# OndrejSladky/kmercamel

Hardware: NVIDIA B200
Metric: distinct k-mers/sec for `compute` (k=31, canonical, device-timed) (higher is better)
Workload: dtype u64

## Files before the change

kmercamel_b200/csrc/engine.cuh:

```cuda
#pragma once
#include "exec.cuh"
#include "kword.cuh"
#include "sort.cuh"
#ifdef KC_HOST_EMUL
#include <algorithm>
#endif

template <int L> struct NodeView {
    const KWord<L> *first;
    const KWord<L> *last;
    u32 n, N;
    int k;
    bool complements;
    KC_HD u32 mirror(u32 v) const { return v < n ? v + n : v - n; }
    KC_HD KWord<L> first_kmer(u32 v) const { return v < n ? first[v] : kmer_reverse_complement(last[v - n], k); }
    KC_HD KWord<L> last_kmer(u32 v) const { return v < n ? last[v] : kmer_reverse_complement(first[v - n], k); }
};

struct PathState {
    u32 *edge_from;
    u32 *edge_to;
    u8 *ovl;
    u32 *chain_head;
    u32 *chain_tail;
};

static const int KC_META_SHIFT = 27;
static const u64 KC_ROLE_P = 1ULL << 36;

template <int L> KC_HD KWord<L + 1> tuple_make(const KWord<L> &key, u64 meta) {
    KWord<L + 1> t;
    t.w[0] = meta << KC_META_SHIFT;
#pragma unroll
    for (int i = 0; i < L; ++i) t.w[i + 1] = key.w[i];
    return t;
}
template <int LT> KC_HD KWord<LT - 1> tuple_key(const KWord<LT> &t) {
    KWord<LT - 1> k;
#pragma unroll
    for (int i = 0; i < LT - 1; ++i) k.w[i] = t.w[i + 1];
    return k;
}
template <int LT> KC_HD bool tuple_is_prefix(const KWord<LT> &t) { return (t.w[0] >> (36 + KC_META_SHIFT)) & 1; }
template <int LT> KC_HD u32 tuple_part(const KWord<LT> &t) { return (u32) (t.w[0] >> (32 + KC_META_SHIFT)) & 15u; }
template <int LT> KC_HD u32 tuple_node(const KWord<LT> &t) {
    u32 id = (u32) (t.w[0] >> KC_META_SHIFT);
    return tuple_is_prefix(t) ? ~id : id;
}

template <int LT> KC_HD u64 tuple_lower_bound(const KWord<LT> *T, u64 lo, u64 hi, const KWord<LT> &probe) {
    while (lo < hi) {
        u64 mid = (lo + hi) >> 1;
        if (T[mid] < probe) lo = mid + 1;
        else hi = mid;
    }
    return lo;
}

#ifdef __CUDACC__
template <int LL> void exec_sort(CudaExec &ex, KWord<LL> *a, KWord<LL> *b, u64 n, int key_bits) { kc_sort<LL>(ex, a, b, n, key_bits); }
#endif
#ifdef KC_HOST_EMUL
template <int LL> void exec_sort(HostExec &, KWord<LL> *a, KWord<LL> *, u64 n, int) {
    std::sort(a, a + n, [](const KWord<LL> &x, const KWord<LL> &y) { return x < y; });
}
#endif

template <int L> struct LevelCtx {
    NodeView<L> nv;
    PathState st;
    const KWord<L + 1> *T;
    u64 nt;
    int d;
    u32 batch;
    u32 *head_w;
    u32 *tail_w;
    u64 *stamp;
    u8 *prim;
    const u8 *ban_flag;
    const u32 *ban_i, *ban_j;
    u32 n_bans;
    bool check_cycles;
};

template <int L> struct SimulatePairFn {
    LevelCtx<L> c;
    const u32 *group_pstart;

    KC_HD bool banned(u32 i, u32 j) const {
        if (!c.ban_flag[i]) return false;
        for (u32 b = 0; b < c.n_bans; ++b)
            if (c.ban_i[b] == i && c.ban_j[b] == j) return true;
        return false;
    }
    KC_HD bool owns_suffix(u32 v, const KWord<L> &ka, const KWord<L> &kb) const {
        if (c.d == 0) return true;
        KWord<L> s = kmer_suffix(c.nv.last_kmer(v), c.d);
        return s == ka || s == kb;
    }
    KC_HD bool owns_prefix(u32 v, const KWord<L> &ka, const KWord<L> &kb) const {
        if (c.d == 0) return true;
        KWord<L> p = kmer_prefix(c.nv.first_kmer(v), c.nv.k, c.d);
        return p == ka || p == kb;
    }
    KC_HD void link(u32 x, u32 y, u64 stampv, u8 primary, const KWord<L> &ka, const KWord<L> &kb) const {
        c.st.edge_from[x] = y;
        c.st.edge_to[y] = x;
        c.st.ovl[x] = (u8) c.d;
        c.stamp[x] = stampv;
        c.prim[x] = primary;
        u32 h = c.head_w[x], t = c.tail_w[y];
        if (owns_suffix(t, ka, kb)) c.head_w[t] = h;
        if (owns_prefix(h, ka, kb)) c.tail_w[h] = t;
    }

    KC_HD void operator()(u64 g) const {
        const KWord<L + 1> *T = c.T;
        const u64 p_beg = group_pstart[g];
        const KWord<L> ka = tuple_key(T[p_beg]);
        KWord<L> kb = ka;
        bool two = false;
        if (c.nv.complements) {
            kb = kmer_reverse_complement(ka, c.d);
            if (kb < ka) return;
            two = kb != ka;
        }
        const u64 meta_max = (1ULL << 37) - 1;
        const u64 s_beg = tuple_lower_bound(T, (u64) 0, p_beg, tuple_make(ka, 0));
        const u64 s_end = p_beg;
        const u64 pa_end = tuple_lower_bound(T, p_beg, c.nt, tuple_make(ka, meta_max));
        u64 s2_beg = 0, s2_end = 0, p2_beg = 0, p2_end = 0;
        if (two) {
            s2_beg = tuple_lower_bound(T, (u64) 0, c.nt, tuple_make(kb, 0));
            s2_end = tuple_lower_bound(T, s2_beg, c.nt, tuple_make(kb, KC_ROLE_P));
            p2_beg = s2_end;
            p2_end = tuple_lower_bound(T, p2_beg, c.nt, tuple_make(kb, meta_max));
        }
        u64 ca = p_beg, cb = p2_beg;
        for (u32 part = 0; part < 16; ++part) {
            u64 ra0 = ca;
            while (ca < pa_end && tuple_part(T[ca]) == part) ++ca;
            u64 ra1 = ca;
            u64 rb0 = cb;
            while (cb < p2_end && tuple_part(T[cb]) == part) ++cb;
            u64 rb1 = cb;
            if (ra0 == ra1 && rb0 == rb1) continue;
            u64 fa = ra0, fb = rb0;
            u64 ia = s_beg, ib = s2_beg;
            while (true) {
                u32 va = (ia < s_end && fa < ra1) ? tuple_node(T[ia]) : KC_NONE;
                u32 vb = (ib < s2_end && fb < rb1) ? tuple_node(T[ib]) : KC_NONE;
                if (va == KC_NONE && vb == KC_NONE) break;
                u32 i;
                u64 *front;
                u64 rend;
                if (va < vb) {
                    i = va;
                    ++ia;
                    front = &fa;
                    rend = ra1;
                } else {
                    i = vb;
                    ++ib;
                    front = &fb;
                    rend = rb1;
                }
                if (c.st.edge_from[i] != KC_NONE) continue;
                while (*front < rend && c.st.edge_to[tuple_node(T[*front])] != KC_NONE) ++*front;
                for (u64 q = *front; q < rend; ++q) {
                    u32 j = tuple_node(T[q]);
                    if (c.st.edge_to[j] != KC_NONE) continue;
                    if (c.check_cycles) {
                        if (c.nv.complements && j == c.nv.mirror(i)) continue;
                        if (j == c.head_w[i]) continue;
                        if (banned(i, j)) continue;
                    }
                    u64 stampv = ((u64) part << 32) | i;
                    link(i, j, stampv, 1, ka, kb);
                    if (c.nv.complements) link(c.nv.mirror(j), c.nv.mirror(i), stampv, 0, ka, kb);
                    break;
                }
            }
        }
    }
};

#ifdef __CUDACC__
#include <cooperative_groups.h>
__global__ void __launch_bounds__(256) kc_doubling_kernel(u32 *jump_a, u32 *jump_b, u32 *fin_a, u32 *fin_b, u64 *max_a, u64 *max_b, u32 ne, int rounds,
                                                          u32 *active , const u32 *ne_dev ) {
    cooperative_groups::grid_group grid = cooperative_groups::this_grid();
    if (ne_dev) ne = *ne_dev;
    u32 *ja = jump_a, *jb = jump_b, *fa = fin_a, *fb = fin_b;
    u64 *ma = max_a, *mb = max_b;
    const u32 stride = gridDim.x * blockDim.x;
    int it = 0;
    for (; it < rounds; ++it) {
        bool any = false;
        for (u32 r = blockIdx.x * blockDim.x + threadIdx.x; r < ne; r += stride) {
            const u32 j = ja[r];
            if (j == KC_NONE) {
                jb[r] = KC_NONE;
                fb[r] = fa[r];
                mb[r] = ma[r];
            } else {
                any = true;
                jb[r] = ja[j];
                fb[r] = fa[j];
                const u64 m1 = ma[r], m2 = ma[j];
                mb[r] = m1 > m2 ? m1 : m2;
            }
        }
        if (__syncthreads_or(any) && threadIdx.x == 0) atomicOr(&active[it % 3], 1u);
        if (blockIdx.x == 0 && threadIdx.x == 0) active[(it + 1) % 3] = 0;
        grid.sync();
        u32 *t = ja; ja = jb; jb = t;
        t = fa; fa = fb; fb = t;
        u64 *m = ma; ma = mb; mb = m;
        const u32 more = *reinterpret_cast<volatile u32 *>(&active[it % 3]);
        if (!more) {
            ++it;
            break;
        }
    }
    if (ja != jump_a) {
        grid.sync();
        for (u32 r = blockIdx.x * blockDim.x + threadIdx.x; r < ne; r += stride) {
            jump_a[r] = ja[r];
            fin_a[r] = fa[r];
            max_a[r] = ma[r];
        }
    }
}
#endif

#include "small_engine.cuh"

struct EngineStats {
    u64 levels_run = 0, tuples_sorted = 0, groups = 0, edges = 0, ban_rounds = 0, bans = 0;
};

template <class Exec, int L> struct Engine {
    Exec &ex;
    NodeView<L> nv;
    PathState st;
    bool strict;
    bool lower_bound;
    bool use_small = true;
    bool fast_levels = true;
    int small_threads_opt = 0;
    EngineStats stats;

    u32 *live_s = nullptr, *live_p = nullptr;
    u32 *list_buf[4] = {nullptr, nullptr, nullptr, nullptr};
    int list_gen = 0;
    u64 n_s = 0, n_p = 0;
    u32 *head_w, *tail_w, *slot_of;
    u64 *stamp;
    u8 *prim, *ban_flag;
    u32 *ban_i, *ban_j, *ban_ctr;
    static const u32 BAN_CAP = 1u << 20;

    Engine(Exec &e, const NodeView<L> &v, bool strict_, bool lower_bound_) : ex(e), nv(v), strict(strict_), lower_bound(lower_bound_) {}

    const u32 *n_dev = nullptr;
    u32 *small_status = nullptr, *small_masks = nullptr;

    void alloc_state() {
        const u64 N = nv.N;
        st.edge_from = ex.template alloc<u32>(N);
        st.edge_to = ex.template alloc<u32>(N);
        st.ovl = ex.template alloc<u8>(N);
        st.chain_head = ex.template alloc<u32>(N);
        st.chain_tail = ex.template alloc<u32>(N);
        head_w = ex.template alloc<u32>(N);
        tail_w = ex.template alloc<u32>(N);
        slot_of = ex.template alloc<u32>(N);
        stamp = ex.template alloc<u64>(N);
        prim = ex.template alloc<u8>(N);
        ban_flag = ex.template alloc<u8>(N);
        ban_i = ex.template alloc<u32>(BAN_CAP);
        ban_j = ex.template alloc<u32>(BAN_CAP);
        ban_ctr = ex.template alloc<u32>(4);
    }

    void init_state() {
        alloc_state();
        const u64 N = nv.N;
        PathState s = st;
        u8 *bf = ban_flag;
        u32 *bc = ban_ctr;
        ex.for_each(N, [=] KC_HD_LAMBDA(u64 v) {
            s.edge_from[v] = KC_NONE;
            s.edge_to[v] = KC_NONE;
            s.ovl[v] = 255;
            bf[v] = 0;
            s.chain_head[v] = (u32) v;
            s.chain_tail[v] = (u32) v;
            if (v < 4) bc[v] = 0;
        });
        if (N < 4) ex.fill_bytes(ban_ctr, 0, 16);
        n_s = n_p = N;
    }

    void run() {
        for (int d = nv.k - 1; d >= 0; --d) {
            const u64 done = lower_bound ? 0 : (nv.complements ? 2 : 1);
            if (n_s <= done) break;
            if (run_small(d)) break;
            run_level(d);
        }
    }

    u32 *small_out = nullptr;
    int small_d = 0;

    void check_small() {
#ifdef __CUDACC__
        if constexpr (Exec::is_device) {
            if (!small_out) return;
            u32 h[KC_SMALL_STATUS_WORDS];
            ex.read_n(small_out, h, KC_SMALL_STATUS_WORDS);
            small_out = nullptr;
            apply_small_status(h);
        }
#endif
    }

    void apply_small_status(const u32 *h) {
        if (std::getenv("KC_TRACE")) {
            std::fprintf(stderr, "[kc_trace] small engine: n_s=%llu n_p=%llu levels=%u groups=%u edges=%u ban_rounds=%u bans=%u; clocks per level (* = run):",
                         (unsigned long long) n_s, (unsigned long long) n_p, h[1], h[2], h[3], h[4], h[5]);
            for (int dd = small_d; dd >= 0; --dd) std::fprintf(stderr, " d%d=%u%s", dd, h[8 + dd] & 0x7FFFFFFFu, (h[8 + dd] >> 31) ? "*" : "");
            std::fprintf(stderr, "; phases: stage+mask=%u tuples=%u sort=%u groups=%u replay=%u validate+commit=%u lists=%u writeback=%u\n", h[136], h[137],
                         h[138], h[139], h[140], h[141], h[142], h[143]);
        }
        if (h[0]) KC_THROW(KC_ERR_INTERNAL, "ban list overflow");
        stats.levels_run += h[1];
        stats.groups += h[2];
        stats.edges += h[3];
        stats.ban_rounds += h[4];
        stats.bans += h[5];
    }

    bool run_small(int d) {
#ifdef __CUDACC__
        if constexpr (Exec::is_device) {
            if (!use_small || lower_bound || n_s + n_p > SmallCfg<L>::T) return false;
            if (!live_s) {
                u32 *a = ex.template alloc<u32>(n_s), *b = ex.template alloc<u32>(n_p);
                ex.for_each(nv.N, [=] KC_HD_LAMBDA(u64 i) {
                    a[i] = (u32) i;
                    b[i] = (u32) i;
                });
                live_s = a;
                live_p = b;
            }
            SmallEngineArgs<L> a;
            a.nv = nv;
            a.st = st;
            a.live_s_a = live_s;
            a.live_p_a = live_p;
            a.live_s_b = ex.template alloc<u32>(n_s);
            a.live_p_b = ex.template alloc<u32>(n_p);
            a.n_s = (u32) n_s;
            a.n_p = (u32) n_p;
            a.head_w = head_w;
            a.tail_w = tail_w;
            a.slot_of = slot_of;
            a.stamp = stamp;
            a.prim = prim;
            a.ban_flag = ban_flag;
            a.ban_i = ban_i;
            a.ban_j = ban_j;
            a.ban_cap = BAN_CAP;
            a.d_start = d;
            a.strict = strict;
            u32 *lvl_mask;
            if (n_dev) {
                a.out = small_status;
                lvl_mask = small_masks;
            } else {
                a.out = ex.template alloc<u32>(KC_SMALL_STATUS_WORDS + kc_small_mask_words(n_s, n_p) + 4 * (n_s + n_p));
                lvl_mask = a.out + KC_SMALL_STATUS_WORDS;
                ex.fill_bytes(a.out, 0, (KC_SMALL_STATUS_WORDS + kc_small_mask_words(n_s, n_p)) * 4);
            }
            a.n_dev = n_dev;
            a.lvl_mask_in = lvl_mask;
            a.end_mask_s_a = lvl_mask + 4;
            a.end_mask_p_a = a.end_mask_s_a + 4 * n_s;
            a.end_mask_s_b = a.end_mask_p_a + 4 * n_p;
            a.end_mask_p_b = a.end_mask_s_b + 4 * n_s;
            const int mask_smem = (int) (SmallCfg<L>::T * sizeof(KWord<L + 1>));
            static KcDevOnce once;
            once.run([&](int) {
                KC_CUDA(cudaFuncSetAttribute(kc_small_engine_kernel<L>, cudaFuncAttributeMaxDynamicSharedMemorySize,
                                             (int) SmallCfg<L>::SMEM));
                KC_CUDA(cudaFuncSetAttribute(kc_small_level_mask_kernel<L>, cudaFuncAttributeMaxDynamicSharedMemorySize, mask_smem));
            });
            {
                typename Exec::Scope sc(ex, KP_SMALL_ENGINE, 0);
                const u32 per_cta = kc_small_mask_levels_per_cta<L>((u32) n_s, (u32) n_p);
                kc_small_level_mask_kernel<L><<<(unsigned) kc_div_up((u64) d + 1, per_cta), 256, mask_smem, ex.stream>>>(nv, live_s, live_p, (u32) n_s, (u32) n_p, d,
                                                                                                                      lvl_mask, a.end_mask_s_a, a.end_mask_p_a, n_dev);
                ++ex.launches;
            }
            {
                typename Exec::Scope sc(ex, KP_SMALL_ENGINE, 0);
                const u64 nt0 = n_s + n_p;
                const unsigned small_threads = small_threads_opt ? (unsigned) small_threads_opt
                                               : n_dev || (nt0 > 128 && nt0 <= 256) || nt0 > 512 ? 512u : 256u;
                kc_small_engine_kernel<L><<<1, small_threads, SmallCfg<L>::SMEM, ex.stream>>>(a);
            }
            ++ex.launches;
            KC_CUDA(cudaGetLastError());
            small_out = n_dev ? nullptr : a.out;
            small_d = d;
            return true;
        }
#endif
        (void) d;
        return false;
    }

    void run_level(int d) {
        typedef KWord<L + 1> TW;
        const u64 nt = n_s + n_p;
        if (n_s == 0 || n_p == 0) return;
        ++stats.levels_run;
        stats.tuples_sorted += nt;
        if (!list_buf[0]) {
            for (int i = 0; i < 4; ++i) list_buf[i] = ex.template alloc<u32>(i < 2 ? n_s : n_p);
        }
        size_t mark = ex.arena->mark();
        TW *T = ex.template alloc<TW>(nt);
        TW *T2 = ex.template alloc<TW>(nt);
        const NodeView<L> v = nv;
        const u32 batch = strict ? nv.N / 16 + 1 : nv.N + 1;
        const u32 *ls = live_s, *lp = live_p;
        const u64 ns = n_s, np = n_p;
        u32 *hw = head_w, *tw = tail_w;
        const PathState s = st;
        ex.for_each(nt, [=] KC_HD_LAMBDA(u64 i) {
            if (i < ns) {
                u32 x = ls ? ls[i] : (u32) i;
                T[i] = tuple_make(kmer_suffix(v.last_kmer(x), d), (u64) x);
                hw[x] = s.chain_head[x];
            } else {
                u32 x = lp ? lp[i - ns] : (u32) (i - ns);
                u64 meta = KC_ROLE_P | ((u64) (x / batch) << 32) | (u64) (u32) ~x;
                T[i] = tuple_make(kmer_prefix(v.first_kmer(x), v.k, d), meta);
                tw[x] = s.chain_tail[x];
            }
        }, KP_TUPLES, nt * (sizeof(KWord<L>) + sizeof(TW)));
        exec_sort<L + 1>(ex, T, T2, nt, 64 + 2 * d);
        u32 *group_pstart = ex.template alloc<u32>(np);
        const TW *Tc = T;
        auto is_group = [=] KC_HD_LAMBDA(u64 i) {
            if (i == 0) return false;
            TW a = Tc[i - 1], b = Tc[i];
            return tuple_is_prefix(b) && !tuple_is_prefix(a) && tuple_key(a) == tuple_key(b);
        };
        auto put_group = [=] KC_HD_LAMBDA(u64 i, u32 r) { group_pstart[r] = (u32) i; };
        LevelCtx<L> c;
        c.nv = nv;
        c.st = st;
        c.T = T;
        c.nt = nt;
        c.d = d;
        c.batch = batch;
        c.head_w = head_w;
        c.tail_w = tail_w;
        c.stamp = stamp;
        c.prim = prim;
        c.ban_flag = ban_flag;
        c.ban_i = ban_i;
        c.ban_j = ban_j;
        c.n_bans = 0;
        c.check_cycles = !lower_bound;
        u32 *new_tail = ex.template alloc<u32>(ns);
        u32 *so = slot_of;
        auto has_edge = [=] KC_HD_LAMBDA(u64 i) { return s.edge_from[ls ? ls[i] : (u32) i] != KC_NONE; };
        auto put_edge = [=] KC_HD_LAMBDA(u64 i, u32 r) {
            u32 x = ls ? ls[i] : (u32) i;
            new_tail[r] = x;
            so[x] = r;
        };
        u64 n_groups = 0, n_edges = 0;
        u32 n_bans = 0;
        bool settled = false, lists_done = false, cycles_pending = false;
#ifdef __CUDACC__
        if constexpr (Exec::is_device) if (fast_levels && (lower_bound || doubling_blocks() > 0)) {
            u64 *cells = ex.template alloc<u64>(6);
            ex.fill_bytes(cells, 0, 40);
            ex.fill_bytes(cells + 5, 0xFF, 8);
            u32 *c_groups = reinterpret_cast<u32 *>(cells), *c_edges = reinterpret_cast<u32 *>(cells + 1);
            u32 *c_ns = reinterpret_cast<u32 *>(cells + 2), *c_np = reinterpret_cast<u32 *>(cells + 3);
            ex.compact_if_nosync(nt, is_group, put_group, c_groups);
            {
                SimulatePairFn<L> sim{c, group_pstart};
                ex.for_each(ns < np ? ns : np, [=] __device__(u64 g) {
                    if (g < *c_groups) sim(g);
                }, KP_SIMULATE);
            }
            ex.compact_if_nosync(ns, has_edge, put_edge, c_edges);
            bool queued = true;
            u32 *jump_a = nullptr, *fin_a = nullptr;
            u64 *max_a = nullptr;
            if (!lower_bound) {
                const u32 ub = (u32) ns;
                jump_a = ex.template alloc<u32>(ub);
                u32 *jump_b = ex.template alloc<u32>(ub);
                fin_a = ex.template alloc<u32>(ub);
                u32 *fin_b = ex.template alloc<u32>(ub);
                max_a = ex.template alloc<u64>(ub);
                u64 *max_b = ex.template alloc<u64>(ub);
                const u64 *stp = stamp;
                u32 *ja = jump_a, *fa = fin_a;
                u64 *ma = max_a;
                ex.for_each(ub, [=] __device__(u64 r) {
                    if (r >= *c_edges) return;
                    u32 x = new_tail[r];
                    u32 t = s.chain_tail[s.edge_from[x]];
                    bool cont = s.edge_from[t] != KC_NONE;
                    ja[r] = cont ? so[t] : KC_NONE;
                    fa[r] = t;
                    ma[r] = stp[x];
                }, KP_DOUBLING, (u64) ub * 36);
                queued = doubling_fused(jump_a, jump_b, fin_a, fin_b, max_a, max_b, ub, kc_ceil_log2(ub) + 1, c_edges);
                if (queued) {
                    ex.for_each(ub, [=] __device__(u64 r) {
                        if (r < *c_edges && ja[r] != KC_NONE) {
                            atomicAdd((kc_ull *) &cells[4], (kc_ull) 1);
                            atomicMin((kc_ull *) &cells[5], (kc_ull) ma[r]);
                        }
                    });
                    ex.for_each(ub, [=] __device__(u64 r) {
                        if (r >= *c_edges || cells[4] != 0) return;
                        u32 x = new_tail[r];
                        u32 h = s.chain_head[x];
                        if (s.edge_to[h] == KC_NONE) {
                            u32 t = fa[r];
                            s.chain_tail[h] = t;
                            s.chain_head[t] = h;
                        }
                    }, KP_COMMIT, (u64) ub * 16);
                }
            }
            if (queued) {
                const u32 *src_s = live_s, *src_p = live_p;
                u32 *dst_s = list_buf[list_gen], *dst_p = list_buf[2 + list_gen];
                ex.compact_if_nosync(ns, [=] __device__(u64 i) { return s.edge_from[src_s ? src_s[i] : (u32) i] == KC_NONE; },
                                     [=] __device__(u64 i, u32 r) { dst_s[r] = src_s ? src_s[i] : (u32) i; }, c_ns);
                ex.compact_if_nosync(np, [=] __device__(u64 i) { return s.edge_to[src_p ? src_p[i] : (u32) i] == KC_NONE; },
                                     [=] __device__(u64 i, u32 r) { dst_p[r] = src_p ? src_p[i] : (u32) i; }, c_np);
                u64 h[5];
                ex.read_n(cells, h, 5);
                n_groups = h[0];
                n_edges = h[1];
                stats.groups += n_groups;
                if (h[4] == 0) {
                    settled = true;
                    if (n_edges) {
                        live_s = dst_s;
                        live_p = dst_p;
                        list_gen ^= 1;
                        n_s = h[2];
                        n_p = h[3];
                    }
                    lists_done = true;
                } else {
                    const u64 *stp = stamp;
                    const u32 *ja = jump_a;
                    const u64 *ma = max_a;
                    const bool only_first = strict;
                    const NodeView<L> v = nv;
                    const u8 *pr = prim;
                    u32 *bi = ban_i, *bj = ban_j, *bc = ban_ctr;
                    u8 *bf = ban_flag;
                    const u32 cap = BAN_CAP;
                    ex.for_each(n_edges, [=] __device__(u64 r) {
                        if (ja[r] == KC_NONE) return;
                        u32 x = new_tail[r];
                        if (stp[x] != ma[r]) return;
                        if (only_first && ma[r] != cells[5]) return;
                        u32 y = s.edge_from[x];
                        u32 pi = x, pj = y;
                        if (!pr[x]) {
                            pi = v.mirror(y);
                            pj = v.mirror(x);
                        }
                        u32 slot = atomicAdd(bc, v.complements ? 2u : 1u);
                        if (slot + 2 <= cap) {
                            bi[slot] = pi;
                            bj[slot] = pj;
                            bf[pi] = 1;
                            if (v.complements) {
                                bi[slot + 1] = v.mirror(pj);
                                bj[slot + 1] = v.mirror(pi);
                                bf[v.mirror(pj)] = 1;
                            }
                        }
                    });
                    cycles_pending = true;
                }
            }
        }
#endif
        if (!settled && !cycles_pending) {
            n_groups = ex.compact_if(nt, is_group, put_group);
            stats.groups += n_groups;
        }
        if (n_groups == 0) {
            ex.arena->release(mark);
            return;
        }
        while (!settled) {
            if (!cycles_pending) {
                c.n_bans = n_bans;
                SimulatePairFn<L> sim{c, group_pstart};
                ex.for_each(n_groups, sim, KP_SIMULATE);
                n_edges = ex.compact_if(ns, has_edge, put_edge);
                if (n_edges == 0 || lower_bound) break;
                if (validate_and_commit(c, new_tail, n_edges, n_bans)) break;
            }
            cycles_pending = false;
            ++stats.ban_rounds;
            n_bans = ex.read(ban_ctr);
            if (n_bans > BAN_CAP) KC_THROW(KC_ERR_INTERNAL, "ban list overflow");
            ex.for_each(nt, [=] KC_HD_LAMBDA(u64 i) {
                if (i < ns) {
                    u32 x = ls ? ls[i] : (u32) i;
                    u32 y = s.edge_from[x];
                    if (y != KC_NONE) {
                        s.edge_to[y] = KC_NONE;
                        s.edge_from[x] = KC_NONE;
                        s.ovl[x] = 255;
                    }
                    hw[x] = s.chain_head[x];
                } else {
                    u32 x = lp ? lp[i - ns] : (u32) (i - ns);
                    tw[x] = s.chain_tail[x];
                }
            });
        }
        if (lower_bound && n_edges) commit_lower_bound();
        stats.edges += n_edges;
        stats.bans += n_bans;
        if (std::getenv("KC_TRACE"))
            std::fprintf(stderr, "[kc_trace] level d=%d: free ends %llu + %llu, groups %llu, edges %llu, bans %u\n", d, (unsigned long long) ns, (unsigned long long) np,
                         (unsigned long long) n_groups, (unsigned long long) n_edges, n_bans);
        if (n_bans) {
            u8 *bf = ban_flag;
            const u32 *bi = ban_i;
            ex.for_each(n_bans, [=] KC_HD_LAMBDA(u64 b) { bf[bi[b]] = 0; });
            ex.fill_bytes(ban_ctr, 0, 16);
        }
        ex.arena->release(mark);
        if (n_edges && !lists_done) {
            const u32 *src_s = live_s, *src_p = live_p;
            u32 *dst_s = list_buf[list_gen], *dst_p = list_buf[2 + list_gen];
            list_gen ^= 1;
            n_s = ex.compact_if(
                ns, [=] KC_HD_LAMBDA(u64 i) { return s.edge_from[src_s ? src_s[i] : (u32) i] == KC_NONE; },
                [=] KC_HD_LAMBDA(u64 i, u32 r) { dst_s[r] = src_s ? src_s[i] : (u32) i; });
            n_p = ex.compact_if(
                np, [=] KC_HD_LAMBDA(u64 i) { return s.edge_to[src_p ? src_p[i] : (u32) i] == KC_NONE; },
                [=] KC_HD_LAMBDA(u64 i, u32 r) { dst_p[r] = src_p ? src_p[i] : (u32) i; });
            live_s = dst_s;
            live_p = dst_p;
        }
    }

#ifdef __CUDACC__
    static int doubling_blocks() {
        static KcDevOnce once;
        static int max_blocks[KC_MAX_DEVICES];
        const int dev = once.run([&](int dv) {
            int coop = 0, per_sm = 0;
            KC_CUDA(cudaDeviceGetAttribute(&coop, cudaDevAttrCooperativeLaunch, dv));
            KC_CUDA(cudaOccupancyMaxActiveBlocksPerMultiprocessor(&per_sm, kc_doubling_kernel, 256, 0));
            max_blocks[dv] = coop ? per_sm * kc_sm_count(dv) : 0;
        });
        return max_blocks[dev];
    }
    bool doubling_fused(u32 *jump_a, u32 *jump_b, u32 *fin_a, u32 *fin_b, u64 *max_a, u64 *max_b, u32 ne, int rounds, const u32 *ne_dev = nullptr) {
        const int max_blocks_dev = doubling_blocks();
        if (max_blocks_dev <= 0) return false;
        u32 *active = ex.template alloc<u32>(4);
        ex.fill_bytes(active, 0, 16);
        u32 blocks = (u32) kc_div_up((u64) ne, 256);
        if (blocks > (u32) max_blocks_dev) blocks = (u32) max_blocks_dev;
        void *args[] = {&jump_a, &jump_b, &fin_a, &fin_b, &max_a, &max_b, &ne, &rounds, &active, &ne_dev};
        typename Exec::Scope sc(ex, KP_DOUBLING, (u64) ne * 32 * 4);
        KC_CUDA(cudaLaunchCooperativeKernel(reinterpret_cast<void *>(kc_doubling_kernel), dim3(blocks), dim3(256), args, 0, ex.stream));
        ++ex.launches;
        return true;
    }
#endif

    bool validate_and_commit(const LevelCtx<L> &c, const u32 *new_tail, u64 n_edges, u32 n_bans_before) {
        size_t mark = ex.arena->mark();
        const u32 ne = (u32) n_edges;
        u32 *jump_a = ex.template alloc<u32>(ne), *jump_b = ex.template alloc<u32>(ne);
        u32 *fin_a = ex.template alloc<u32>(ne), *fin_b = ex.template alloc<u32>(ne);
        u64 *max_a = ex.template alloc<u64>(ne), *max_b = ex.template alloc<u64>(ne);
        const PathState s = st;
        const u32 *so = slot_of;
        const u64 *stp = stamp;
        ex.for_each(ne, [=] KC_HD_LAMBDA(u64 r) {
            u32 x = new_tail[r];
            u32 t = s.chain_tail[s.edge_from[x]];
            bool cont = s.edge_from[t] != KC_NONE;
            jump_a[r] = cont ? so[t] : KC_NONE;
            fin_a[r] = t;
            max_a[r] = stp[x];
        }, KP_DOUBLING, (u64) ne * 36);
        int rounds = kc_ceil_log2(ne) + 1;
        bool fused = false;
#ifdef __CUDACC__
        if constexpr (Exec::is_device) fused = doubling_fused(jump_a, jump_b, fin_a, fin_b, max_a, max_b, ne, rounds);
#endif
        for (int it = 0; it < rounds && !fused; ++it) {
            const u32 *ja = jump_a, *fa = fin_a;
            const u64 *ma = max_a;
            u32 *jb = jump_b, *fb = fin_b;
            u64 *mb = max_b;
            ex.for_each(ne, [=] KC_HD_LAMBDA(u64 r) {
                u32 j = ja[r];
                if (j == KC_NONE) {
                    jb[r] = KC_NONE;
                    fb[r] = fa[r];
                    mb[r] = ma[r];
                } else {
                    jb[r] = ja[j];
                    fb[r] = fa[j];
                    u64 m1 = ma[r], m2 = ma[j];
                    mb[r] = m1 > m2 ? m1 : m2;
                }
            }, KP_DOUBLING, (u64) ne * 32);
            u32 *t = jump_a; jump_a = jump_b; jump_b = t;
            t = fin_a; fin_a = fin_b; fin_b = t;
            u64 *m = max_a; max_a = max_b; max_b = m;
        }
        u64 *cell = ex.template alloc<u64>(2);
        ex.fill_bytes(cell, 0, 8);
        ex.fill_bytes(cell + 1, 0xFF, 8);
        {
            const u32 *ja = jump_a;
            const u64 *ma = max_a;
            ex.for_each(ne, [=] KC_HD_LAMBDA(u64 r) {
                if (ja[r] != KC_NONE) {
                    KC_ATOMIC_ADD((kc_ull *) &cell[0], (kc_ull) 1);
                    KC_ATOMIC_MIN((kc_ull *) &cell[1], (kc_ull) ma[r]);
                }
            });
        }
        u64 n_cyc = ex.read(cell);
        if (n_cyc == 0) {
            const u32 *fa = fin_a;
            ex.for_each(ne, [=] KC_HD_LAMBDA(u64 r) {
                u32 x = new_tail[r];
                u32 h = s.chain_head[x];
                if (s.edge_to[h] == KC_NONE) {
                    u32 t = fa[r];
                    s.chain_tail[h] = t;
                    s.chain_head[t] = h;
                }
            }, KP_COMMIT, (u64) ne * 16);
            ex.arena->release(mark);
            return true;
        }
        {
            const u32 *ja = jump_a;
            const u64 *ma = max_a;
            const bool only_first = strict;
            const NodeView<L> v = nv;
            const u8 *pr = prim;
            u32 *bi = ban_i, *bj = ban_j, *bc = ban_ctr;
            u8 *bf = ban_flag;
            const u32 cap = BAN_CAP;
            ex.for_each(ne, [=] KC_HD_LAMBDA(u64 r) {
                if (ja[r] == KC_NONE) return;
                u32 x = new_tail[r];
                if (stp[x] != ma[r]) return;
                if (only_first && ma[r] != cell[1]) return;
                u32 y = s.edge_from[x];
                u32 pi = x, pj = y;
                if (!pr[x]) {
                    pi = v.mirror(y);
                    pj = v.mirror(x);
                }
                u32 slot = KC_ATOMIC_ADD(bc, v.complements ? 2u : 1u);
                if (slot + 2 <= cap) {
                    bi[slot] = pi;
                    bj[slot] = pj;
                    bf[pi] = 1;
                    if (v.complements) {
                        bi[slot + 1] = v.mirror(pj);
                        bj[slot + 1] = v.mirror(pi);
                        bf[v.mirror(pj)] = 1;
                    }
                }
            });
        }
        (void) n_bans_before;
        ex.arena->release(mark);
        return false;
    }

    void commit_lower_bound() {}
};
```

kmercamel_b200/csrc/small_engine.cuh:

```cuda
#pragma once

static const u32 KC_SMALL_STATUS_WORDS = 8 + 128 + 8;
KC_HD u64 kc_small_mask_words(u64 n_s, u64 n_p) { return 4 + 4 * (n_s + n_p); }

#ifdef __CUDACC__

template <int L> struct SmallCfg {
    static constexpr u32 T = L <= 2 ? 4096 : 2048;
    static constexpr u32 H = T / 2;
    static constexpr u32 NS = 1024;
    static constexpr u32 RANK_SORT = 384;
    static constexpr bool STAGE_KMERS = false;
    static constexpr size_t SMEM = (size_t) T * sizeof(KWord<L + 1>) + (size_t) H * (4 * 6 + 8 * 2) + (size_t) NS * (8 + 4 * 7 + 3) +
                                   (STAGE_KMERS ? (size_t) NS * 2 * sizeof(KWord<L>) + 16 : 0);
};

template <int L> struct SmallEngineArgs {
    NodeView<L> nv;
    PathState st;
    u32 *live_s_a, *live_p_a, *live_s_b, *live_p_b;
    u32 n_s, n_p;
    u32 *head_w, *tail_w, *slot_of;
    u64 *stamp;
    u8 *prim, *ban_flag;
    u32 *ban_i, *ban_j;
    u32 ban_cap;
    int d_start;
    bool strict;
    u32 *out;
    const u32 *lvl_mask_in;
    u32 *end_mask_s_a, *end_mask_p_a, *end_mask_s_b, *end_mask_p_b;
    const u32 *n_dev;
};

static const u32 KC_SMALL_MASK_LEVELS = 2;
template <int L> KC_HD u32 kc_small_mask_table_slots(u32 n_p) {
    u32 H2 = 64;
    while (H2 < 2 * n_p) H2 <<= 1;
    return H2;
}
template <int L> KC_HD u32 kc_small_mask_levels_per_cta(u32 n_s, u32 n_p) {
    const u32 avail = (u32) ((SmallCfg<L>::T * sizeof(KWord<L + 1>) - (size_t) (n_s + n_p) * sizeof(KWord<L>)) / 4);
    u32 G = avail / kc_small_mask_table_slots<L>(n_p);
    if (G > KC_SMALL_MASK_LEVELS) G = KC_SMALL_MASK_LEVELS;
    return G < 1 ? 1 : G;
}

template <int L>
__global__ void __launch_bounds__(256) kc_small_level_mask_kernel(NodeView<L> v, const u32 *__restrict__ ls, const u32 *__restrict__ lp, u32 n_s, u32 n_p,
                                                                  int d_start, u32 *mask_out , u32 *end_mask_s ,
                                                                  u32 *end_mask_p , const u32 *n_dev ) {
    extern __shared__ __align__(16) unsigned char kc_smem_raw[];
    __shared__ u32 s_hits;
    const u32 tid = threadIdx.x, NT = blockDim.x;
    const u32 G = kc_small_mask_levels_per_cta<L>(n_s, n_p);
    if (n_dev) {
        v.n = n_dev[0];
        v.N = n_dev[1];
        n_s = n_p = v.N;
    }
    KWord<L> *pk = reinterpret_cast<KWord<L> *>(kc_smem_raw), *sk = pk + n_p;
    u32 *tab = reinterpret_cast<u32 *>(sk + n_s);
    const u32 H2 = kc_small_mask_table_slots<L>(n_p);
    const int d_hi = d_start - (int) (blockIdx.x * G);
    if (d_hi < 0) return;
    const u32 g = (u32) (d_hi + 1) < G ? (u32) (d_hi + 1) : G;
    for (u32 i = tid; i < n_p; i += NT) pk[i] = v.first_kmer(lp[i]);
    for (u32 i = tid; i < n_s; i += NT) sk[i] = v.last_kmer(ls[i]);
    for (u32 i = tid; i < g * H2; i += NT) tab[i] = KC_NONE;
    if (tid == 0) s_hits = 0;
    __syncthreads();
    for (u32 item = tid; item < g * n_p; item += NT) {
        const u32 lev = item / n_p, i = item - lev * n_p;
        const int d = d_hi - (int) lev;
        u32 *tb = tab + lev * H2;
        const KWord<L> key = kmer_prefix(pk[i], v.k, d);
        u64 h = 0;
#pragma unroll
        for (int q = 0; q < L; ++q) h = (h ^ key.w[q]) * 0x9E3779B97F4A7C15ULL;
        u32 sl = (u32) (h >> 40) & (H2 - 1);
        while (true) {
            const u32 old = atomicCAS(&tb[sl], KC_NONE, i);
            if (old == KC_NONE || kmer_prefix(pk[old], v.k, d) == key) break;
            sl = (sl + 1) & (H2 - 1);
        }
    }
    __syncthreads();
    constexpr u32 PROBED = 0x80000000u;
    u32 hits = 0;
    for (u32 item = tid; item < g * n_s; item += NT) {
        const u32 lev = item / n_s, i = item - lev * n_s;
        const int d = d_hi - (int) lev;
        u32 *tb = tab + lev * H2;
        const KWord<L> key = kmer_suffix(sk[i], d);
        u64 h = 0;
#pragma unroll
        for (int q = 0; q < L; ++q) h = (h ^ key.w[q]) * 0x9E3779B97F4A7C15ULL;
        u32 sl = (u32) (h >> 40) & (H2 - 1);
        while (true) {
            const u32 o = tb[sl];
            if (o == KC_NONE) break;
            if (kmer_prefix(pk[o & ~PROBED], v.k, d) == key) {
                hits |= 1u << lev;
                if (!(o & PROBED)) tb[sl] = o | PROBED;
                atomicOr(&end_mask_s[4 * i + ((u32) d >> 5)], 1u << (d & 31));
                break;
            }
            sl = (sl + 1) & (H2 - 1);
        }
    }
    if (hits) atomicOr(&s_hits, hits);
    __syncthreads();
    if (tid == 0) {
        const u32 hm = s_hits;
        for (u32 lev = 0; lev < g; ++lev)
            if ((hm >> lev) & 1u) atomicOr(&mask_out[(d_hi - (int) lev) >> 5], 1u << ((d_hi - (int) lev) & 31));
    }
    const u32 hm = s_hits;
    for (u32 item = tid; item < g * n_p; item += NT) {
        const u32 lev = item / n_p, i = item - lev * n_p;
        if (!((hm >> lev) & 1u)) continue;
        const int d = d_hi - (int) lev;
        const u32 *tb = tab + lev * H2;
        const KWord<L> key = kmer_prefix(pk[i], v.k, d);
        u64 h = 0;
#pragma unroll
        for (int q = 0; q < L; ++q) h = (h ^ key.w[q]) * 0x9E3779B97F4A7C15ULL;
        u32 sl = (u32) (h >> 40) & (H2 - 1);
        while (true) {
            const u32 o = tb[sl];
            if (kmer_prefix(pk[o & ~PROBED], v.k, d) == key) {
                if (o & PROBED) atomicOr(&end_mask_p[4 * i + ((u32) d >> 5)], 1u << (d & 31));
                break;
            }
            sl = (sl + 1) & (H2 - 1);
        }
    }
}

template <int L> __global__ void __launch_bounds__(512) kc_small_engine_kernel(SmallEngineArgs<L> a) {
    typedef KWord<L + 1> TW;
    constexpr u32 TCAP = SmallCfg<L>::T, HCAP = SmallCfg<L>::H;
    extern __shared__ __align__(16) unsigned char kc_smem_raw[];
    TW *const T0 = reinterpret_cast<TW *>(kc_smem_raw);
    TW *T = T0;
    u64 *max0 = reinterpret_cast<u64 *>(T0 + TCAP);
    u64 *max1 = max0 + HCAP;
    u32 *group_pstart = reinterpret_cast<u32 *>(max1 + HCAP);
    u32 *new_tail = group_pstart + HCAP;
    u32 *jump0 = new_tail + HCAP, *jump1 = jump0 + HCAP, *fin0 = jump1 + HCAP, *fin1 = fin0 + HCAP;
    __shared__ u32 s_groups, s_edges, s_cyc, s_bans, s_live_s, s_live_p;
    __shared__ u32 lvl_mask[4];
    __shared__ kc_ull s_min;
    const u32 tid = threadIdx.x;
    const u32 NT = blockDim.x;
    NodeView<L> v = a.nv;
    if (a.n_dev) {
        v.n = a.n_dev[0];
        v.N = a.n_dev[1];
    }
    PathState s = a.st;
    u32 *head_w = a.head_w, *tail_w = a.tail_w, *slot_of = a.slot_of;
    u64 *stamp = a.stamp;
    u8 *prim = a.prim, *ban_flag = a.ban_flag;
    const bool local_state = v.N <= SmallCfg<L>::NS;
    if (local_state) {
        constexpr u32 NS = SmallCfg<L>::NS;
        u64 *l_stamp = reinterpret_cast<u64 *>(fin1 + HCAP);
        u32 *l32 = reinterpret_cast<u32 *>(l_stamp + NS);
        u8 *l8 = reinterpret_cast<u8 *>(l32 + 7 * NS);
        for (u32 i = tid; i < v.N; i += NT) {
            l32[i] = s.edge_from[i];
            l32[NS + i] = s.edge_to[i];
            l32[2 * NS + i] = s.chain_head[i];
            l32[3 * NS + i] = s.chain_tail[i];
            l8[i] = s.ovl[i];
            l8[2 * NS + i] = 0;
        }
        s.edge_from = l32;
        s.edge_to = l32 + NS;
        s.chain_head = l32 + 2 * NS;
        s.chain_tail = l32 + 3 * NS;
        head_w = l32 + 4 * NS;
        tail_w = l32 + 5 * NS;
        slot_of = l32 + 6 * NS;
        stamp = l_stamp;
        s.ovl = l8;
        prim = l8 + NS;
        ban_flag = l8 + 2 * NS;
        if constexpr (SmallCfg<L>::STAGE_KMERS) {
            KWord<L> *lk = reinterpret_cast<KWord<L> *>((reinterpret_cast<uintptr_t>(l8 + 3 * NS) + 15) & ~(uintptr_t) 15);
            for (u32 i = tid; i < v.n; i += NT) {
                lk[i] = a.nv.first[i];
                lk[NS + i] = a.nv.last[i];
            }
            v.first = lk;
            v.last = lk + NS;
        }
        __syncthreads();
    }
    u32 n_s = a.n_dev ? v.N : a.n_s, n_p = a.n_dev ? v.N : a.n_p;
    u32 *ls = a.live_s_a, *lp = a.live_p_a, *ls2 = a.live_s_b, *lp2 = a.live_p_b;
    u32 *ms = a.end_mask_s_a, *mp = a.end_mask_p_a, *ms2 = a.end_mask_s_b, *mp2 = a.end_mask_p_b;
    __shared__ u32 s_nt;
    const u32 batch = a.strict ? v.N / 16 + 1 : v.N + 1;
    const u32 done = v.complements ? 2u : 1u;
    u32 st_levels = 0, st_groups = 0, st_edges = 0, st_rounds = 0, st_bans = 0;
    long long ph[8] = {0, 0, 0, 0, 0, 0, 0, 0};
    long long ph_t = clock64();
#define KC_PH(i) do { const long long kc_now = clock64(); ph[i] += kc_now - ph_t; ph_t = kc_now; } while (0)

    if (tid < 4) lvl_mask[tid] = a.lvl_mask_in[tid];
    __syncthreads();

    KC_PH(0);
    for (int d = a.d_start; d >= 0; --d) {
        if (n_s <= done || n_p == 0) break;
        const long long lvl_t0 = clock64();
        if (!((lvl_mask[d >> 5] >> (d & 31)) & 1u)) continue;
        ++st_levels;
        const u32 n_live = n_s + n_p;
        T = T0;
        if (tid == 0) {
            s_nt = 0;
            s_groups = 0;
            s_bans = 0;
        }
        __syncthreads();
        for (u32 i = tid; i < n_live; i += NT) {
            if (i < n_s) {
                u32 x = ls[i];
                head_w[x] = s.chain_head[x];
                if ((ms[4 * i + ((u32) d >> 5)] >> (d & 31)) & 1u) T[atomicAdd(&s_nt, 1u)] = tuple_make(kmer_suffix(v.last_kmer(x), d), (u64) x);
            } else {
                u32 x = lp[i - n_s];
                tail_w[x] = s.chain_tail[x];
                if ((mp[4 * (i - n_s) + ((u32) d >> 5)] >> (d & 31)) & 1u) {
                    u64 meta = KC_ROLE_P | ((u64) (x / batch) << 32) | (u64) (u32) ~x;
                    T[atomicAdd(&s_nt, 1u)] = tuple_make(kmer_prefix(v.first_kmer(x), v.k, d), meta);
                }
            }
        }
        for (u32 i = tid; i < n_live && i <= SmallCfg<L>::RANK_SORT; i += NT) group_pstart[i] = 0;
        __syncthreads();
        const u32 nt = s_nt;
        KC_PH(1);
        if (nt <= SmallCfg<L>::RANK_SORT) {
            TW *dst = T0 + HCAP;
            const u32 P = nt ? (NT / nt < 8u ? NT / nt : 8u) : 0u;
            if (P >= 2) {
                u32 *rk = group_pstart;
                if (tid < nt * P) {
                    const u32 part = tid / nt, i = tid - part * nt;
                    const u32 j0 = part * nt / P, j1 = (part + 1) * nt / P;
                    const TW mine = T0[i];
                    u32 r = 0;
#pragma unroll 8
                    for (u32 j = j0; j < j1; ++j) r += T0[j] < mine ? 1u : 0u;
                    atomicAdd(&rk[i], r);
                }
                __syncthreads();
                for (u32 i = tid; i < nt; i += NT) dst[rk[i]] = T0[i];
            } else {
                for (u32 i = tid; i < nt; i += NT) {
                    const TW mine = T0[i];
                    u32 r = 0;
#pragma unroll 8
                    for (u32 j = 0; j < nt; ++j) r += T0[j] < mine ? 1u : 0u;
                    dst[r] = mine;
                }
            }
            T = dst;
            __syncthreads();
        } else {
            kc_block_bitonic<L + 1>(T, nt, NT);
        }
        KC_PH(2);
        for (u32 i = tid + 1; i < nt; i += NT) {
            TW p = T[i - 1], q = T[i];
            if (tuple_is_prefix(q) && !tuple_is_prefix(p) && tuple_key(p) == tuple_key(q)) group_pstart[atomicAdd(&s_groups, 1u)] = i;
        }
        __syncthreads();
        const u32 n_groups = s_groups;
        st_groups += n_groups;
        KC_PH(3);
        if (n_groups) {
            LevelCtx<L> c;
            c.nv = v;
            c.st = s;
            c.T = T;
            c.nt = nt;
            c.d = d;
            c.batch = batch;
            c.head_w = head_w;
            c.tail_w = tail_w;
            c.stamp = stamp;
            c.prim = prim;
            c.ban_flag = ban_flag;
            c.ban_i = a.ban_i;
            c.ban_j = a.ban_j;
            c.check_cycles = true;
            u32 n_bans = 0;
            while (true) {
                c.n_bans = n_bans;
                SimulatePairFn<L> sim{c, group_pstart};
                for (u32 g = tid; g < n_groups; g += NT) sim((u64) g);
                if (tid == 0) {
                    s_edges = 0;
                    s_cyc = 0;
                    s_min = ~0ULL;
                }
                __syncthreads();
                KC_PH(4);
                for (u32 i = tid; i < n_s; i += NT) {
                    u32 x = ls[i];
                    if (s.edge_from[x] != KC_NONE) {
                        u32 r = atomicAdd(&s_edges, 1u);
                        new_tail[r] = x;
                        slot_of[x] = r;
                    }
                }
                __syncthreads();
                const u32 ne = s_edges;
                if (ne == 0) break;
                for (u32 r = tid; r < ne; r += NT) {
                    u32 x = new_tail[r];
                    u32 t = s.chain_tail[s.edge_from[x]];
                    bool cont = s.edge_from[t] != KC_NONE;
                    jump0[r] = cont ? slot_of[t] : KC_NONE;
                    fin0[r] = t;
                    max0[r] = stamp[x];
                }
                __syncthreads();
                u32 *ja = jump0, *jb = jump1, *fa = fin0, *fb = fin1;
                u64 *ma = max0, *mb = max1;
                int rounds = 1;
                while ((1u << (rounds - 1)) < ne) ++rounds;
                for (int it = 0; it < rounds; ++it) {
                    for (u32 r = tid; r < ne; r += NT) {
                        u32 j = ja[r];
                        if (j == KC_NONE) {
                            jb[r] = KC_NONE;
                            fb[r] = fa[r];
                            mb[r] = ma[r];
                        } else {
                            jb[r] = ja[j];
                            fb[r] = fa[j];
                            u64 m1 = ma[r], m2 = ma[j];
                            mb[r] = m1 > m2 ? m1 : m2;
                        }
                    }
                    __syncthreads();
                    u32 *t32 = ja; ja = jb; jb = t32;
                    t32 = fa; fa = fb; fb = t32;
                    u64 *t64 = ma; ma = mb; mb = t64;
                }
                for (u32 r = tid; r < ne; r += NT)
                    if (ja[r] != KC_NONE) {
                        atomicAdd(&s_cyc, 1u);
                        atomicMin(&s_min, (kc_ull) ma[r]);
                    }
                __syncthreads();
                if (s_cyc == 0) {
                    for (u32 r = tid; r < ne; r += NT) {
                        u32 x = new_tail[r];
                        u32 h = s.chain_head[x];
                        if (s.edge_to[h] == KC_NONE) {
                            u32 t = fa[r];
                            s.chain_tail[h] = t;
                            s.chain_head[t] = h;
                        }
                    }
                    st_edges += ne;
                    __syncthreads();
                    break;
                }
                const kc_ull first_stamp = s_min;
                for (u32 r = tid; r < ne; r += NT) {
                    if (ja[r] == KC_NONE) continue;
                    u32 x = new_tail[r];
                    if (stamp[x] != ma[r]) continue;
                    if (a.strict && ma[r] != first_stamp) continue;
                    u32 y = s.edge_from[x];
                    u32 pi = x, pj = y;
                    if (!prim[x]) {
                        pi = v.mirror(y);
                        pj = v.mirror(x);
                    }
                    u32 slot = atomicAdd(&s_bans, v.complements ? 2u : 1u);
                    if (slot + 2 <= a.ban_cap) {
                        a.ban_i[slot] = pi;
                        a.ban_j[slot] = pj;
                        ban_flag[pi] = 1;
                        if (v.complements) {
                            a.ban_i[slot + 1] = v.mirror(pj);
                            a.ban_j[slot + 1] = v.mirror(pi);
                            ban_flag[v.mirror(pj)] = 1;
                        }
                    }
                }
                __syncthreads();
                n_bans = s_bans;
                ++st_rounds;
                if (n_bans + 2 > a.ban_cap) {
                    if (tid == 0) a.out[0] = 1;
                    return;
                }
                for (u32 i = tid; i < n_live; i += NT) {
                    if (i < n_s) {
                        u32 x = ls[i];
                        u32 y = s.edge_from[x];
                        if (y != KC_NONE) {
                            s.edge_to[y] = KC_NONE;
                            s.edge_from[x] = KC_NONE;
                            s.ovl[x] = 255;
                        }
                        head_w[x] = s.chain_head[x];
                    } else {
                        u32 x = lp[i - n_s];
                        tail_w[x] = s.chain_tail[x];
                    }
                }
                __syncthreads();
            }
            for (u32 b = tid; b < n_bans; b += NT) ban_flag[a.ban_i[b]] = 0;
            st_bans += n_bans;
            KC_PH(5);
        }
        if (tid == 0) {
            s_live_s = 0;
            s_live_p = 0;
        }
        __syncthreads();
        for (u32 i = tid; i < n_s; i += NT) {
            u32 x = ls[i];
            if (s.edge_from[x] == KC_NONE) {
                const u32 to = atomicAdd(&s_live_s, 1u);
                ls2[to] = x;
                *reinterpret_cast<uint4 *>(ms2 + 4 * to) = *reinterpret_cast<const uint4 *>(ms + 4 * i);
            }
        }
        for (u32 i = tid; i < n_p; i += NT) {
            u32 x = lp[i];
            if (s.edge_to[x] == KC_NONE) {
                const u32 to = atomicAdd(&s_live_p, 1u);
                lp2[to] = x;
                *reinterpret_cast<uint4 *>(mp2 + 4 * to) = *reinterpret_cast<const uint4 *>(mp + 4 * i);
            }
        }
        __syncthreads();
        n_s = s_live_s;
        n_p = s_live_p;
        u32 *t32 = ls; ls = ls2; ls2 = t32;
        t32 = lp; lp = lp2; lp2 = t32;
        t32 = ms; ms = ms2; ms2 = t32;
        t32 = mp; mp = mp2; mp2 = t32;
        __syncthreads();
        KC_PH(6);
        if (tid == 0) a.out[8 + d] = (u32) (clock64() - lvl_t0) | 0x80000000u;
    }
    if (local_state) {
        __syncthreads();
        for (u32 i = tid; i < v.N; i += NT) {
            a.st.edge_from[i] = s.edge_from[i];
            a.st.edge_to[i] = s.edge_to[i];
            a.st.chain_head[i] = s.chain_head[i];
            a.st.chain_tail[i] = s.chain_tail[i];
            a.st.ovl[i] = s.ovl[i];
        }
    }
    KC_PH(7);
    if (tid == 0) {
        for (int i = 0; i < 8; ++i) a.out[8 + 128 + i] = (u32) ph[i];
        a.out[1] = st_levels;
        a.out[2] = st_groups;
        a.out[3] = st_edges;
        a.out[4] = st_rounds;
        a.out[5] = st_bans;
    }
}

#undef KC_PH

#endif
```

Baseline: 79.93 billion.

## Replay pair groups with warp-cooperative scans and precomputed group bounds

The single-thread-per-group pair simulation in the small engine is replaced with a tiled replay. Group range bounds are precomputed once per ban round into scratch buffers, along with per-node suffix/prefix position tables. Groups with many ends are then replayed by a full warp using ballots to find the run ends and the first free partner, while small groups keep one thread each. The aim is to cut serial per-thread scanning and repeated binary searches, at the cost of extra shared scratch reuse, extra syncs, and more complex ownership checks.

```diff
diff --git a/kmercamel_b200/csrc/engine.cuh b/kmercamel_b200/csrc/engine.cuh
--- a/kmercamel_b200/csrc/engine.cuh
+++ b/kmercamel_b200/csrc/engine.cuh
@@ -184,6 +184,132 @@
         }
     }
 };
+
+#ifdef __CUDACC__
+template <int L> struct SimulatePairTile {
+    LevelCtx<L> c;
+    const u32 *s_beg, *p_beg, *p_end, *s2_beg, *p2_beg, *p2_end;
+    const u16 *spos, *ppos;
+
+    __device__ u32 pair_ends(u32 g) const { return s_beg[g] == KC_NONE ? 0u : p_end[g] - s_beg[g] + p2_end[g] - s2_beg[g]; }
+
+    template <u32 W> __device__ static u32 tile_mask() {
+        return W == 32 ? ~0u : ((1u << (W & 31)) - 1) << ((threadIdx.x & 31u) & ~(W - 1));
+    }
+    template <u32 W> __device__ static u32 ballot(bool p) {
+        const u32 m = tile_mask<W>();
+        return (__ballot_sync(m, p) & m) >> ((threadIdx.x & 31u) & ~(W - 1));
+    }
+
+    __device__ bool owns_suffix(u32 v, u32 g, const KWord<L> &ka, const KWord<L> &kb) const {
+        if (c.d == 0) return true;
+        if (!spos) return SimulatePairFn<L>{c, nullptr}.owns_suffix(v, ka, kb);
+        const u32 q = spos[v];
+        if (q >= c.nt || tuple_is_prefix(c.T[q]) || tuple_node(c.T[q]) != v) return false;
+        return (q >= s_beg[g] && q < p_beg[g]) || (q >= s2_beg[g] && q < p2_beg[g]);
+    }
+    __device__ bool owns_prefix(u32 v, u32 g, const KWord<L> &ka, const KWord<L> &kb) const {
+        if (c.d == 0) return true;
+        if (!ppos) return SimulatePairFn<L>{c, nullptr}.owns_prefix(v, ka, kb);
+        const u32 q = ppos[v];
+        if (q >= c.nt || !tuple_is_prefix(c.T[q]) || tuple_node(c.T[q]) != v) return false;
+        return (q >= p_beg[g] && q < p_end[g]) || (q >= p2_beg[g] && q < p2_end[g]);
+    }
+    __device__ void link(u32 x, u32 y, u64 stampv, u8 primary, u32 g, const KWord<L> &ka, const KWord<L> &kb) const {
+        c.st.edge_from[x] = y;
+        c.st.edge_to[y] = x;
+        c.st.ovl[x] = (u8) c.d;
+        c.stamp[x] = stampv;
+        c.prim[x] = primary;
+        u32 h = c.head_w[x], t = c.tail_w[y];
+        if (owns_suffix(t, g, ka, kb)) c.head_w[t] = h;
+        if (owns_prefix(h, g, ka, kb)) c.tail_w[h] = t;
+    }
+    template <u32 W> __device__ u32 run_end(u32 cur, u32 end, u32 part, u32 lane) const {
+        while (true) {
+            const u32 q = cur + lane;
+            const u32 m = ballot<W>(q >= end || tuple_part(c.T[q]) != part);
+            if (m) return cur + __ffs(m) - 1;
+            cur += W;
+        }
+    }
+
+    template <u32 W> __device__ void replay(u32 g, u32 lane) const {
+        const KWord<L + 1> *T = c.T;
+        const u32 sa = s_beg[g];
+        if (sa == KC_NONE) return;
+        const u32 pa = p_beg[g], pa_end = p_end[g], sb = s2_beg[g], pb = p2_beg[g], pb_end = p2_end[g];
+        const KWord<L> ka = tuple_key(T[pa]);
+        const KWord<L> kb = c.nv.complements ? kmer_reverse_complement(ka, c.d) : ka;
+        u32 ca = pa, cb = pb;
+        while (true) {
+            const u32 part_a = ca < pa_end ? tuple_part(T[ca]) : 16u, part_b = cb < pb_end ? tuple_part(T[cb]) : 16u;
+            const u32 part = part_a < part_b ? part_a : part_b;
+            if (part == 16u) break;
+            const u32 ra0 = ca, ra1 = part_a == part ? run_end<W>(ca, pa_end, part, lane) : ca;
+            const u32 rb0 = cb, rb1 = part_b == part ? run_end<W>(cb, pb_end, part, lane) : cb;
+            ca = ra1;
+            cb = rb1;
+            u32 fa = ra0, fb = rb0;
+            u32 ia = sa, ib = sb;
+            while (true) {
+                const u32 va = (ia < pa && fa < ra1) ? tuple_node(T[ia]) : KC_NONE;
+                const u32 vb = (ib < pb && fb < rb1) ? tuple_node(T[ib]) : KC_NONE;
+                if (va == KC_NONE && vb == KC_NONE) break;
+                u32 i, *front, rend;
+                if (va < vb) {
+                    i = va;
+                    ++ia;
+                    front = &fa;
+                    rend = ra1;
+                } else {
+                    i = vb;
+                    ++ib;
+                    front = &fb;
+                    rend = rb1;
+                }
+                if (c.st.edge_from[i] != KC_NONE) continue;
+                const u32 hw = c.check_cycles ? c.head_w[i] : KC_NONE;
+                const bool ban_i = c.check_cycles && c.ban_flag[i];
+                const u32 mi = c.nv.complements ? c.nv.mirror(i) : KC_NONE;
+                bool front_found = false;
+                for (u32 base = *front; base < rend; base += W) {
+                    const u32 q = base + lane;
+                    const u32 j = q < rend ? tuple_node(T[q]) : KC_NONE;
+                    const bool free = j != KC_NONE && c.st.edge_to[j] == KC_NONE;
+                    bool ok = free;
+                    if (ok && c.check_cycles) {
+                        if (j == mi || j == hw) ok = false;
+                        else if (ban_i) {
+                            for (u32 b = 0; b < c.n_bans; ++b)
+                                if (c.ban_i[b] == i && c.ban_j[b] == j) {
+                                    ok = false;
+                                    break;
+                                }
+                        }
+                    }
+                    const u32 fm = ballot<W>(free || q >= rend), om = ballot<W>(ok);
+                    if (!front_found) {
+                        front_found = fm != 0;
+                        *front = fm ? base + __ffs(fm) - 1 : base + W;
+                    }
+                    if (om) {
+                        u32 jj = j;
+                        if constexpr (W > 1) jj = __shfl_sync(tile_mask<W>(), j, __ffs(om) - 1, W);
+                        if (lane == 0) {
+                            const u64 stampv = ((u64) part << 32) | i;
+                            link(i, jj, stampv, 1, g, ka, kb);
+                            if (c.nv.complements) link(c.nv.mirror(jj), c.nv.mirror(i), stampv, 0, g, ka, kb);
+                        }
+                        if constexpr (W > 1) __syncwarp(tile_mask<W>());
+                        break;
+                    }
+                }
+            }
+        }
+    }
+};
+#endif
 
 #ifdef __CUDACC__
 #include <cooperative_groups.h>
diff --git a/kmercamel_b200/csrc/small_engine.cuh b/kmercamel_b200/csrc/small_engine.cuh
--- a/kmercamel_b200/csrc/small_engine.cuh
+++ b/kmercamel_b200/csrc/small_engine.cuh
@@ -300,11 +300,62 @@
             c.ban_i = a.ban_i;
             c.ban_j = a.ban_j;
             c.check_cycles = true;
+            SimulatePairTile<L> sim;
+            sim.c = c;
+            u32 *const gb = reinterpret_cast<u32 *>(max0);
+            u32 *const g_sbeg = gb, *const g_pend = gb + HCAP, *const g_s2beg = gb + 2 * HCAP, *const g_p2beg = gb + 3 * HCAP;
+            u32 *const g_p2end = new_tail;
+            u16 *const spos = local_state ? reinterpret_cast<u16 *>(jump0) : nullptr;
+            u16 *const ppos = spos ? spos + SmallCfg<L>::NS : nullptr;
+            static_assert(2 * SmallCfg<L>::NS * sizeof(u16) <= HCAP * sizeof(u32), "end positions must fit in jump0");
+            sim.s_beg = g_sbeg;
+            sim.p_beg = group_pstart;
+            sim.p_end = g_pend;
+            sim.s2_beg = g_s2beg;
+            sim.p2_beg = g_p2beg;
+            sim.p2_end = g_p2end;
+            sim.spos = spos;
+            sim.ppos = ppos;
             u32 n_bans = 0;
             while (true) {
-                c.n_bans = n_bans;
-                SimulatePairFn<L> sim{c, group_pstart};
-                for (u32 g = tid; g < n_groups; g += NT) sim((u64) g);
+                for (u32 g = tid; g < n_groups; g += NT) {
+                    const u32 p_beg = group_pstart[g];
+                    const KWord<L> ka = tuple_key(T[p_beg]);
+                    KWord<L> kb = ka;
+                    if (v.complements) {
+                        kb = kmer_reverse_complement(ka, d);
+                        if (kb < ka) {
+                            g_sbeg[g] = KC_NONE;
+                            continue;
+                        }
+                    }
+                    const u64 meta_max = (1ULL << 37) - 1;
+                    g_sbeg[g] = (u32) tuple_lower_bound(T, (u64) 0, (u64) p_beg, tuple_make(ka, 0));
+                    g_pend[g] = (u32) tuple_lower_bound(T, (u64) p_beg, (u64) nt, tuple_make(ka, meta_max));
+                    u32 s2 = 0, p2 = 0, p2e = 0;
+                    if (kb != ka) {
+                        s2 = (u32) tuple_lower_bound(T, (u64) 0, (u64) nt, tuple_make(kb, 0));
+                        p2 = (u32) tuple_lower_bound(T, (u64) s2, (u64) nt, tuple_make(kb, KC_ROLE_P));
+                        p2e = (u32) tuple_lower_bound(T, (u64) p2, (u64) nt, tuple_make(kb, meta_max));
+                    }
+                    g_s2beg[g] = s2;
+                    g_p2beg[g] = p2;
+                    g_p2end[g] = p2e;
+                }
+                if (spos)
+                    for (u32 i = tid; i < nt; i += NT) {
+                        const TW t = T[i];
+                        (tuple_is_prefix(t) ? ppos : spos)[tuple_node(t)] = (u16) i;
+                    }
+                __syncthreads();
+                constexpr u32 WIDE = 16;
+                sim.c.n_bans = n_bans;
+                for (u32 g = tid / 32; g < n_groups; g += NT / 32)
+                    if (sim.pair_ends(g) > WIDE) sim.template replay<32>(g, tid % 32);
+                for (u32 g = tid; g < n_groups; g += NT) {
+                    const u32 e = sim.pair_ends(g);
+                    if (e && e <= WIDE) sim.template replay<1>(g, 0);
+                }
                 if (tid == 0) {
                     s_edges = 0;
                     s_cyc = 0;
diff --git a/profiles/engine_phases.py b/profiles/engine_phases.py
--- /dev/null
+++ b/profiles/engine_phases.py
@@ -0,0 +1,97 @@
+import argparse
+import json
+import os
+import re
+import subprocess
+import sys
+import tempfile
+
+ROOT = os.path.dirname(os.path.dirname(os.path.abspath(__file__)))
+sys.path.insert(0, ROOT)
+os.environ["KC_TRACE"] = "1"
+
+PHASES = ["stage+mask", "tuples", "sort", "groups", "replay", "validate+commit", "lists", "writeback"]
+LINE = re.compile(r"small engine: n_s=(\d+) n_p=(\d+) levels=(\d+) groups=(\d+) edges=(\d+) ban_rounds=(\d+) bans=(\d+); "
+                  r"clocks per level \(\* = run\):(.*); phases: (.*)$")
+
+
+def parse(line):
+    m = LINE.search(line)
+    if not m:
+        return None
+    levels = {}
+    for tok in m.group(8).split():
+        name, val = tok.split("=")
+        if val.endswith("*"):
+            levels[int(name[1:])] = int(val[:-1])
+    phases = {}
+    for tok in m.group(9).split():
+        name, val = tok.split("=")
+        phases[name] = int(val)
+    keys = ["n_s", "n_p", "levels", "groups", "edges", "ban_rounds", "bans"]
+    out = {kk: int(m.group(i + 1)) for i, kk in enumerate(keys)}
+    out["level_clocks"] = {f"d{d}": c for d, c in sorted(levels.items(), reverse=True)}
+    out["phase_clocks"] = phases
+    out["total_clocks"] = sum(phases.values())
+    return out
+
+
+def main():
+    ap = argparse.ArgumentParser()
+    ap.add_argument("--out", required=True)
+    ap.add_argument("--label", default="")
+    ap.add_argument("--reps", type=int, default=5)
+    args = ap.parse_args()
+    import torch
+    import kmercamel_b200 as kb
+    from kmercamel_b200 import synth
+
+    os.makedirs(args.out, exist_ok=True)
+    gpu = subprocess.run(["nvidia-smi", "-i", "0", "--query-gpu=name,power.limit,clocks.max.sm", "--format=csv,noheader"],
+                         capture_output=True, text=True).stdout.strip()
+    inputs = [("configs[1] 50 x 1 Mbp", synth.random_genome_records(50, 1_000_000, 12345))]
+    inputs += [(f"{n} x 40 kbp", synth.random_genome_records(n, 40_000, 500 + n)) for n in (100, 200, 400)]
+    ctx = kb.Context(0, torch.cuda.current_stream().cuda_stream)
+    results = []
+    for name, recs in inputs:
+        d = torch.from_numpy(synth.frame_records(recs)[0]).cuda()
+        for _ in range(2):
+            ctx.compute_device(d.data_ptr(), d.numel(), k=31)
+        torch.cuda.synchronize()
+        ctx.profile_enable(True)
+        ctx.profile_reset()
+        sys.stderr.flush()
+        saved = os.dup(2)
+        with tempfile.TemporaryFile(mode="w+") as tf:
+            os.dup2(tf.fileno(), 2)
+            try:
+                for _ in range(args.reps):
+                    ctx.compute_device(d.data_ptr(), d.numel(), k=31)
+                torch.cuda.synchronize()
+            finally:
+                os.dup2(saved, 2)
+                os.close(saved)
+            tf.seek(0)
+            runs = [p for p in (parse(ln) for ln in tf) if p]
+        prof = ctx.profile()
+        ctx.profile_enable(False)
+        assert len(runs) == args.reps, f"{name}: {len(runs)} trace lines for {args.reps} runs"
+        last = runs[-1]
+        runs.sort(key=lambda r: r["total_clocks"])
+        med = runs[len(runs) // 2]
+        med["input"] = name
+        med["small_engine_ms_per_call"] = round(prof["small_engine"]["ms"] / args.reps, 4)
+        med["total_clocks_all_runs"] = sorted(r["total_clocks"] for r in runs)
+        assert last["edges"] == med["edges"]
+        results.append(med)
+        ph = med["phase_clocks"]
+        print(f"{name:24s} engine {med['small_engine_ms_per_call']:.4f} ms  levels {med['levels']:2d} groups {med['groups']:4d} "
+              f"edges {med['edges']:4d} bans {med['bans']:3d}  " + " ".join(f"{k}={ph.get(k, 0)}" for k in PHASES), flush=True)
+    ctx.close()
+    fn = os.path.join(args.out, f"engine_phases{'_' + args.label if args.label else ''}.json")
+    json.dump({"gpu": gpu, "label": args.label, "inputs": results}, open(fn, "w"), indent=1)
+    print("wrote", fn)
+
+
+if __name__ == "__main__":
+    main()
```

New measurement: 76.86 billion (median of 6 runs). 0.962x the previous value.
